# agussomacal/ROMHighContrast

Hardware: AMD Instinct MI355X
Metric: snapshot_solves_per_sec (higher is better)
Workload: dtype f64

## Files before the change

romhighcontrast_amd/csrc/rom_fem_kernels.hip:

```cpp
#include "rom_fem_dev.h"

__global__ void k_build_A0(double* A0, const double* Qp, const double* rho, int n1, int n1p, int N) {
  size_t idx = blockIdx.x * size_t(blockDim.x) + threadIdx.x;
  size_t total = size_t(n1) * n1 * n1p;
  if (idx >= total) return;
  int m = int(idx % n1p);
  size_t ij = idx / n1p;
  int j = int(ij % n1) + 1, i = int(ij / n1) + 1;
  A0[idx] = (m < n1) ? Qp[size_t(j - 1) * n1p + m] * rho[size_t(m) * (N + 1) + i] : 0.0;
}

__global__ void k_repack_table(const double* __restrict__ G, int ld, int nseg, int n1, int orient, double* __restrict__ Gs) {
  const long long idx = blockIdx.x * (long long)blockDim.x + threadIdx.x;
  const long long hrows = (long long)n1 * n1;
  if (idx >= (long long)nseg * hrows * 8) return;
  const int kk = int(idx & 7);
  const long long rp = (idx >> 3) % hrows, seg = (idx >> 3) / hrows;
  const long long row = orient ? (rp % n1) * n1 + rp / n1 : rp;
  const int k = int(seg) * 8 + kk;
  Gs[idx] = k < ld ? G[row * ld + k] : 0.0;
}

__global__ void k_mask_table(double* __restrict__ G, int ld, int n1, ExtThresholds th) {
  const long long idx = blockIdx.x * (long long)blockDim.x + threadIdx.x;
// ... 854 lines not shown
  const int m_raw = 4 * int(blockIdx.x) + w;
  const bool live = m_raw < Mc;
  const int m = live ? m_raw : Mc - 1;
  const double* am = a + size_t(m) * f.kblk;
  double* ym = f.y + size_t(m) * f.nGp;
#ifdef ROMHC_SOLVE1_STAMPS
  unsigned long long stamp[10];
#define S1_STAMP(i) stamp[i] = __builtin_readcyclecounter()
  S1_STAMP(0);
#else
#define S1_STAMP(i)
#endif
#define S1_WAVE_SYNC()                                   \
  do {                                                   \
    asm volatile("s_waitcnt lgkmcnt(0)" ::: "memory");   \
    __builtin_amdgcn_wave_barrier();                     \
  } while (0)
#define S1_BARRIER() asm volatile("s_waitcnt lgkmcnt(0)\n\ts_barrier" ::: "memory")
  const int l16 = lane & 15, l4 = lane >> 4;

  if (upd) {
    int4 irec[6], crec[S1_ITEM_PASSES];
    int wd[DENSE_GROUPS_MAX];
    {
      const int4* ir = reinterpret_cast<const int4*>(f.s1_items) + size_t(min(lane, max(f.ndi, 1) - 1)) * 6;
#pragma unroll
      for (int x = 0; x < 6; ++x) irec[x] = ir[x];
#pragma unroll
      for (int r = 0; r < S1_ITEM_PASSES; ++r) crec[r] = reinterpret_cast<const int4*>(f.s1_citems)[min(lane + 64 * r, max(f.ncoef, 1) - 1)];
#pragma unroll
      for (int g = 0; g < DENSE_GROUPS_MAX; ++g) wd[g] = g < f.ndg ? f.dweight[g * 64 + lane] : -2;
    }
    const int xr_first = lane < f.ncross ? f.xred[lane] : 0;
    const int2 sc_b = lane < f.nsc ? reinterpret_cast<const int2*>(f.scb)[lane] : int2{0, 0};
    const RhsTerm rt = f.rhs[min(lane, max(f.nrhs, 1) - 1)];
    const double gvec = f.g[lane];
    __syncthreads();
    {
      const double rcoef = lane < f.nrhs ? (rt.kind == 0 ? aL[rt.b0] / (aL[rt.e0] + aL[rt.e1]) : 0.5) : 0.0;
      double y = gvec;
      for (int t0 = 0; t0 < f.nrhs; t0 += 8) {
        double rv[8];
#pragma unroll
        for (int x = 0; x < 8; ++x) {
          rv[x] = 0.0;
          if (t0 + x < f.nrhs) {
            const int pos = __builtin_amdgcn_readlane(rt.pos, t0 + x), len = __builtin_amdgcn_readlane(rt.len, t0 + x);
            const int voff = __builtin_amdgcn_readlane(rt.voff, t0 + x);
            if (lane >= pos && lane < pos + len) rv[x] = f.vec[voff + lane - pos];
          }
        }
#pragma unroll
        for (int x = 0; x < 8; ++x)
          if (t0 + x < f.nrhs) y += readlane_f64(rcoef, t0 + x) * rv[x];
      }
      zs[lane] = y;
    }
    if (live)
      for (int i = lane; i < f.nGp; i += 64) ym[i] = 0.0;
    if (live && lane < f.nsc) ym[f.spos0 + lane] = sc_b.y >= 0 ? 1.0 / (aL[sc_b.x] + aL[sc_b.y]) : (1.0 / (double(f.N) * double(f.N))) / aL[sc_b.x];
    for (int i = lane + 64; live && i < f.nsc; i += 64) {
      const int b0 = f.scb[2 * i], b1 = f.scb[2 * i + 1];
      ym[f.spos0 + i] = b1 >= 0 ? 1.0 / (aL[b0] + aL[b1]) : (1.0 / (double(f.N) * double(f.N))) / aL[b0];
    }
    double wgt[DENSE_GROUPS_MAX];
#pragma unroll
    for (int g = 0; g < DENSE_GROUPS_MAX; ++g) {
      wgt[g] = 0.0;
      if (g < f.ndg) {
        const DenseGroup& dg = f.dgroups[g];
        wgt[g] = wd[g] >= 0 ? aL[wd[g]] : (wd[g] == -1 ? (aL[dg.b0] + aL[dg.b1]) / 2 : 0.0);
      }
    }
    const bool has_it = lane < f.ndi;
    const int it_g = irec[0].x, it_pos = irec[0].y, it_nv = irec[0].z;
    double it_den = 1.0, it_cv[4] = {0.0, 0.0, 0.0, 0.0}, it_vv[4] = {0.0, 0.0, 0.0, 0.0};
    if (has_it) {
      const int voff[4] = {irec[1].y, irec[1].z, irec[1].w, irec[2].x}, vblk[4] = {irec[2].y, irec[2].z, irec[2].w, irec[3].x};
      const int vu0[4] = {irec[3].y, irec[3].z, irec[3].w, irec[4].x}, vu1[4] = {irec[4].y, irec[4].z, irec[4].w, irec[5].x};
      it_den = aL[irec[0].w] + aL[irec[1].x];
#pragma unroll
      for (int v = 0; v < 4; ++v)
        if (v < it_nv) {
          it_cv[v] = aL[vblk[v]] / (aL[vu0[v]] + aL[vu1[v]]);
          it_vv[v] = f.vec[voff[v]];
        }
    }
    int ci_dst[S1_ITEM_PASSES], ci_src[S1_ITEM_PASSES];
#pragma unroll
    for (int r = 0; r < S1_ITEM_PASSES; ++r) {
      ci_src[r] = -1;
      ci_dst[r] = crec[r].x & 0xfffffff;
      if (lane + 64 * r < f.ncoef) {
        const int code = crec[r].x >> 28;
        if (code == 2) ci_src[r] = crec[r].y;
        else if (code != 0 && live) ym[ci_dst[r]] = code == 1 ? 1.0 / (aL[crec[r].z] + aL[crec[r].w]) : 0.0;
      }
    }
    __syncthreads();
    d4_t C[4][4];
    {
      int q = 0;
#pragma unroll
      for (int ib = 0; ib < 4; ++ib)
#pragma unroll
        for (int jb = 0; jb <= ib; ++jb, ++q)
#pragma unroll
          for (int g = 0; g < 4; ++g) {
            const int R = 16 * ib + 4 * g + l4, Cc = 16 * jb + l16;
            const double x = Ls[(q * 4 + g) * 64 + lane];
            C[ib][jb][g] = (R >= f.s1_ndr || Cc >= f.s1_ndr) ? (R == Cc ? 1.0 : 0.0) : x;
          }
    }
#pragma unroll
    for (int x = 0; x < 8; ++x) PnB[x * 64 + lane] = 0.0;
    S1_BARRIER();
#ifdef ROMHC_SOLVE1_PANEL_STAMPS
    unsigned long long uwait = 0;
    const unsigned long long ut0 = __builtin_readcyclecounter();
#endif
#pragma unroll
    for (int p = 0; p < 15; ++p) {
      const int jb = p >> 2;
      {
        const int p1 = p + 1, jb1 = p1 >> 2, co1 = 4 * (p1 & 3);
        double* dstp = PnB + (p1 & 1) * 256;
        if ((l16 >> 2) == (p1 & 3)) {
#pragma unroll
          for (int ib = jb1; ib < 4; ++ib)
#pragma unroll
            for (int g = 0; g < 4; ++g) dstp[(16 * ib + 4 * g + l4) * 4 + (l16 - co1)] = C[ib][jb1][g];
        }
      }
#ifdef ROMHC_SOLVE1_PANEL_STAMPS
      { const unsigned long long t0_ = __builtin_readcyclecounter(); S1_BARRIER(); uwait += __builtin_readcyclecounter() - t0_; }
#else
      S1_BARRIER();
#endif
      const double* Pp = (p & 1) ? Pn1 : Pn;
      double frag[4];
#pragma unroll
      for (int x = jb; x < 4; ++x) frag[x] = Pp[(16 * x + l16) * 4 + l4];
#pragma unroll
      for (int jb2 = jb; jb2 < 4; ++jb2)
#pragma unroll
        for (int ib = jb2; ib < 4; ++ib)
          C[ib][jb2] = __builtin_amdgcn_mfma_f64_16x16x4f64(-frag[ib], frag[jb2], C[ib][jb2], 0, 0, 0);
    }
#ifdef ROMHC_SOLVE1_PANEL_STAMPS
    const unsigned long long ut1 = __builtin_readcyclecounter();
#endif
    S1_BARRIER();
    if (!live) return;
    const double z = zs[lane];
    ym[lane] = z;
    if (lane < f.ncross) ym[f.xb0 + lane] = zs[xr_first];
    for (int x = lane + 64; x < f.ncross; x += 64) ym[f.xb0 + x] = zs[f.xred[x]];
#pragma unroll
    for (int g = 0; g < DENSE_GROUPS_MAX; ++g)
      if (g < f.ndg) wz[g * 64 + lane] = wgt[g] * z;
    S1_WAVE_SYNC();
    if (has_it) {
      const double* wg = wz + it_g * 64;
      const double* D = Dl + lane;
      double acc = 0.0;
#pragma unroll 1
      for (int j0 = 0; j0 < 64; j0 += 16) {
#pragma unroll
        for (int j = 0; j < 16; ++j) acc += D[(j0 + j) * f.ndi] * wg[j0 + j];
      }
#pragma unroll
      for (int v = 0; v < 4; ++v)
        if (v < it_nv) acc += it_cv[v] * it_vv[v];
      ym[it_pos] = acc / it_den;
    }
#pragma unroll
    for (int r = 0; r < S1_ITEM_PASSES; ++r)
      if (ci_src[r] >= 0) ym[ci_dst[r]] = zs[ci_src[r]];
    for (int it = lane + 64 * S1_ITEM_PASSES; it < f.ncoef; it += 64) {
      const CoefGroup& cg = f.groups[f.item_group[it]];
      const int k = f.item_k[it];
      if (cg.kind == 1 && k < cg.r) continue;
      ym[cg.cpos + k] = k == cg.r ? 1.0 / (aL[cg.b0] + aL[cg.b1]) : (k < cg.r ? zs[cg.zpos + k] : 0.0);
    }
#ifdef ROMHC_SOLVE1_STAMPS
    if (lane < 12) ym[lane] = PnB[lane];
#ifdef ROMHC_SOLVE1_PANEL_STAMPS
    if (lane == 12) ym[12] = double(uwait);
    if (lane == 13) ym[13] = double(ut1 - ut0);
#endif
#endif
    return;
  }

  {
    const unsigned d0 = unsigned(size_t((__attribute__((address_space(3))) char*)s1_dyn)) + unsigned(S1_COEF_BYTES + 4 * S1_WAVE_BYTES);
    const int nchunk = (f.ndi + 1) >> 1;
    const char* src = reinterpret_cast<const char*>(f.dmat);
    for (int c = w; c < nchunk; c += 4)
      asm volatile("s_mov_b32 m0, %0\n\tglobal_load_lds_dwordx4 %1, %2" ::"s"(__builtin_amdgcn_readfirstlane(d0 + unsigned(c) * 1024u)),
                   "v"(unsigned(lane) * 16u), "s"(x128_uniform(src + size_t(c) * 1024))
                   : "memory", "m0");
  }
  {
    const int p0 = f.wp0[w], np = f.wp0[w + 1] - p0;
    const double2* pbase = reinterpret_cast<const double2*>(f.pool_acc) + size_t(p0) * 128 + lane;
    double2 v[PAIR_RING][2];
    auto issue = [&](int i, double2 (&dst)[2]) {
      dst[0] = pbase[size_t(i) * 128];
      dst[1] = pbase[size_t(i) * 128 + 64];
    };
    const double a_l = lane < f.kblk ? am[lane] : 1.0;
    const GenTerm gt = f.terms[f.s1_t0 + min(lane, f.s1_nterm - 1)];
    int mine = f.wmeta[p0 + lane];
#pragma unroll
    for (int u = 0; u < PAIR_RING; ++u) issue(u, v[u]);
#pragma unroll
    for (int x = 0; x < 40; ++x) Ls[x * 64 + lane] = 0.0;
    aL[lane] = a_l;
    S1_WAVE_SYNC();
    coefs[w * 64 + lane] = lane < f.s1_nterm ? term_coef(gt, aL) : 0.0;
    __syncthreads();
    double cf[4];
#pragma unroll
    for (int s = 0; s < 4; ++s) cf[s] = coefs[s * 64 + lane];
    double acc4[4][4];
#pragma unroll
    for (int s = 0; s < 4; ++s)
#pragma unroll
      for (int g = 0; g < 4; ++g) acc4[s][g] = 0.0;
    double* const Cl0 = reinterpret_cast<double*>(s1_dyn + S1_COEF_BYTES) + lane;
    S1_STAMP(1);
    for (int base = 0; base < np; base += 64) {
      const int cur = mine;
      const int nxt = f.wmeta[p0 + base + 64 + lane];
      const int cnt = min(64, np - base);
#pragma unroll
      for (int i0 = 0; i0 < 64; i0 += PAIR_RING) {
        if (i0 >= cnt) break;
#pragma unroll
        for (int u = 0; u < PAIR_RING; ++u) {
          const int i = i0 + u;
          const int meta = __builtin_amdgcn_readlane(cur, i);
#pragma unroll
          for (int s = 0; s < 4; ++s) {
            const double c = readlane_f64(cf[s], meta & 0xff);
            acc4[s][0] = __builtin_fma(c, v[u][0].x, acc4[s][0]);
            acc4[s][1] = __builtin_fma(c, v[u][0].y, acc4[s][1]);
            acc4[s][2] = __builtin_fma(c, v[u][1].x, acc4[s][2]);
            acc4[s][3] = __builtin_fma(c, v[u][1].y, acc4[s][3]);
          }
          if (meta >> 16) {
            double* dst = Cl0 + ((meta >> 8) & 0xff) * 256;
#pragma unroll
            for (int s = 0; s < 4; ++s)
#pragma unroll
              for (int g = 0; g < 4; ++g) {
                dst[s * (S1_WAVE_BYTES / 8) + g * 64] = acc4[s][g];
                acc4[s][g] = 0.0;
              }
          }
          issue(base + i + PAIR_RING, v[u]);
        }
      }
      mine = nxt;
    }
    asm volatile("s_waitcnt vmcnt(0)" ::: "memory");
    __syncthreads();
  }
  S1_STAMP(2);
  double nv[4];
  {
    const int ib = lane >> 4;
    const double* src = Ls + ((ib * (ib + 1) / 2) * 4 + ((lane >> 2) & 3)) * 64 + (lane & 3) * 16;
    const double2 x0 = *reinterpret_cast<const double2*>(src), x1 = *reinterpret_cast<const double2*>(src + 2);
    nv[0] = x0.x; nv[1] = x0.y; nv[2] = x1.x; nv[3] = x1.y;
#pragma unroll
    for (int k = 0; k < 4; ++k)
      if (lane >= f.s1_ndr || k >= f.s1_ndr) nv[k] = lane == k ? 1.0 : 0.0;
  }
  S1_BARRIER();
  S1_STAMP(3);
  double y = zs[lane];
  double myrs = 0.0;
#ifdef ROMHC_SOLVE1_PANEL_STAMPS
  unsigned long long fwait = 0;
#endif
  S1_STAMP(4);
#pragma unroll
  for (int p = 0; p < 16; ++p) {
    const int c0 = 4 * p;
    chol_panel_regs(lane, c0, nv, y, myrs);
    {
      double* Pp = (p & 1) ? Pn1 : Pn;
      *reinterpret_cast<double2*>(&Pp[lane * 4]) = double2{nv[0], nv[1]};
      *reinterpret_cast<double2*>(&Pp[lane * 4 + 2]) = double2{nv[2], nv[3]};
    }
    if ((lane >> 2) >= p) {
      double* lrow = Ls + s1_lrow(lane) + c0;
      *reinterpret_cast<double2*>(lrow) = double2{nv[0], nv[1]};
      *reinterpret_cast<double2*>(lrow + 2) = double2{nv[2], nv[3]};
    }
    if (p < 15) {
#ifdef ROMHC_SOLVE1_PANEL_STAMPS
      { const unsigned long long t0_ = __builtin_readcyclecounter(); S1_BARRIER(); fwait += __builtin_readcyclecounter() - t0_; }
#else
      S1_BARRIER();
#endif
      const double* bp = PnB + ((p + 1) & 1) * 256 + lane * 4;
      const double2 b01 = *reinterpret_cast<const double2*>(bp), b23 = *reinterpret_cast<const double2*>(bp + 2);
      double nn[4] = {b01.x, b01.y, b23.x, b23.y};
#pragma unroll
      for (int kk = 0; kk < 4; ++kk)
#pragma unroll
        for (int k = 0; k < 4; ++k) nn[kk] = __builtin_fma(-nv[k], readlane_f64(nv[k], c0 + 4 + kk), nn[kk]);
#pragma unroll
      for (int kk = 0; kk < 4; ++kk) nv[kk] = nn[kk];
    }
  }
  if (chol_pivots_bad(myrs) && live && lane == 0) atomicOr(f.status, 1);
  S1_WAVE_SYNC();
  S1_STAMP(5);
#pragma unroll
  for (int h = 1; h >= 0; --h) {
    double lcol[32];
#pragma unroll
    for (int j = 0; j < 32; ++j) lcol[j] = Ls[s1_lrow(32 * h + j) + lane];
#pragma unroll
    for (int j = 31; j >= 0; --j) {
      const int jj = 32 * h + j;
      const double xj = readlane_f64(y, jj) * readlane_f64(myrs, jj);
      if (lane == jj) y = xj;
      else if (lane < jj) y -= lcol[j] * xj;
    }
  }
  zs[lane] = y;
  S1_STAMP(6);
#ifdef ROMHC_SOLVE1_STAMPS
#pragma unroll
  for (int k = 0; k < 7; ++k)
    if (lane == k) PnB[k] = double(stamp[k] - stamp[0]);
  if (lane >= 7 && lane < 12) PnB[lane] = 0.0;
#ifdef ROMHC_SOLVE1_PANEL_STAMPS
  if (lane == 10) PnB[10] = double(fwait);
#endif
#endif
  S1_BARRIER();
#undef S1_STAMP
#undef S1_WAVE_SYNC
#undef S1_BARRIER
}

template <int NS>
__device__ inline void panel_body(const FemDev& f, const double* __restrict__ am0, int m0, int nsys, int j, int ent, double* lds,
                                  double* yj, double* coef) {
  double* Cb = lds;
  double* stB = lds + TILE_DOUBLES;
  const int slot = f.colrow[ent];
  const int ti = f.colti[ent];
  const WavePos wp;
  const TileDesc& d = f.desc[slot];
  const int t = threadIdx.x;
  const bool stream = NS == 1 && f.tile_stream && d.t1 - d.t0 <= 128;
  STile st[NS];
  if (!stream) s_tile_load<NS>(st, d, f, am0, nsys, coef);
  static_assert(TD_LDS_BYTES <= FACT_LDS_DOUBLES * 8, "the DMA slots alias the staging area and the C tile");
#pragma unroll
  for (int q = 0; q < NS; ++q) {
    if (q >= nsys) break;
    const int m = m0 + q;
    double* Lm = f.L + size_t(m) * f.nslots * 4096;
    if (q > 0) __syncthreads();
    if (t < 64) yj[t] = f.y[size_t(m) * f.nGp + j * 64 + t];
    TileStream<1> ts;
    if (stream) s_tile_stream_begin<1>(ts, slot, d, f, am0 + size_t(q) * f.kblk, 1);
    Acc acc;
    acc_zero(acc);
    accumulate_klist_dma(f, slot, Lm, [](int) { return true; }, acc, reinterpret_cast<char*>(lds), wp);
    if (stream) {
      __syncthreads();
      double* T[1] = {Cb};
      s_tile_to_lds<1>(T, ts, d, f);
      tile_minus_acc(Cb, acc, wp);
    } else {
      tile_from_acc(Cb, acc, st[q], wp);
    }

    acc_zero(acc);
    const double* I = f.invL + (size_t(m) * f.T + j) * 4096 + (t >> 2) * 64 + (t & 3) * 2;
    const int kmax = (wp.wc + 1) * 32;
    {
      const int fr = wp.lane & 15, kq = wp.lane >> 4;
      double2 vb = *reinterpret_cast<const double2*>(I);
      for (int ch = 0; ch < 8; ++ch) {
        *reinterpret_cast<double2*>(stB + (t >> 2) * LDK8 + (t & 3) * 2) = vb;
        __syncthreads();
        if (ch + 1 < 8) vb = *reinterpret_cast<const double2*>(I + (ch + 1) * 8);
        if (ch * 8 < kmax) {
          const double* pa = Cb + (wp.wr * 32 + fr) * LDC + ch * 8 + kq;
          const double* pb = stB + (wp.wc * 32 + fr) * LDK8 + kq;
#pragma unroll
          for (int kk = 0; kk < 8; kk += 4) {
            const double a0 = pa[kk], a1 = pa[16 * LDC + kk];
            const double b0 = pb[kk], b1 = pb[16 * LDK8 + kk];
            acc.c[0][0] = __builtin_amdgcn_mfma_f64_16x16x4f64(a0, b0, acc.c[0][0], 0, 0, 0);
            acc.c[0][1] = __builtin_amdgcn_mfma_f64_16x16x4f64(a0, b1, acc.c[0][1], 0, 0, 0);
            acc.c[1][0] = __builtin_amdgcn_mfma_f64_16x16x4f64(a1, b0, acc.c[1][0], 0, 0, 0);
            acc.c[1][1] = __builtin_amdgcn_mfma_f64_16x16x4f64(a1, b1, acc.c[1][1], 0, 0, 0);
          }
        }
        __syncthreads();
      }
    }

    double* Lout = Lm + size_t(slot) * 4096;
#pragma unroll
    for (int i = 0; i < 2; ++i)
#pragma unroll
      for (int jb = 0; jb < 2; ++jb)
#pragma unroll
        for (int g = 0; g < 4; ++g) {
          int r = acc_row(wp, i, g), c = acc_col(wp, jb);
          double v = acc.c[i][jb][g];
          Lout[r * 64 + c] = v;
          Cb[r * LDC + c] = v;
        }
    __syncthreads();
    if (t < 64) {
      double sum = 0.0;
      for (int k = 0; k < 64; ++k) sum += Cb[t * LDC + k] * yj[k];
      f.y[size_t(m) * f.nGp + ti * 64 + t] -= sum;
    }
  }
}

__device__ inline void panel_block(int b, int nrows, int Mc, int& m, int& row) {
  const int xcd = b & 7, idx = b >> 3;
  const int full = (Mc >> 3) << 3;
  m = xcd + 8 * (idx / nrows);
  row = idx % nrows;
  if (m >= full) {
    const int tb = b - full * nrows;
    m = full + tb / nrows;
    row = tb % nrows;
  }
}

template <int NS>
__global__ __launch_bounds__(256, 4) void k_factor_panel(FemDev f, const double* __restrict__ a, int j, int Mc) {
  __shared__ __align__(16) double lds[FACT_LDS_DOUBLES];
  __shared__ double yj[64];
  double* coef = lds;
  int mp, row;
  panel_block(blockIdx.x, f.colptr[j + 1] - f.colptr[j], (Mc + NS - 1) / NS, mp, row);
  const int m0 = mp * NS;
  panel_body<NS>(f, a + size_t(m0) * f.kblk, m0, min(NS, Mc - m0), j, f.colptr[j] + row, lds, yj, coef);
}
template __global__ void k_factor_panel<1>(FemDev, const double*, int, int);

__global__ __launch_bounds__(256) void k_backsolve(FemDev f) {
  extern __shared__ __align__(16) double xs[];
  __shared__ double red[4][64];
  __shared__ double vs[64];
  const int m = blockIdx.x;
  const int t = threadIdx.x, c = t & 63, part = t >> 6;
  const double* Lm = f.L + size_t(m) * f.nslots * 4096;
  double* ym = f.y + size_t(m) * f.nGp;
  for (int j = f.T - 1; j >= 0; --j) {
    double s = 0.0;
    for (int e = f.colptr[j]; e < f.colptr[j + 1]; ++e) {
      const double* Lt = Lm + size_t(f.colrow[e]) * 4096;
      const double* xi = xs + f.colti[e] * 64;
#pragma unroll 4
      for (int rr = part * 16; rr < part * 16 + 16; ++rr) s += Lt[rr * 64 + c] * xi[rr];
    }
    red[part][c] = s;
    __syncthreads();
    if (t < 64) vs[t] = ym[j * 64 + t] - (red[0][t] + red[1][t] + red[2][t] + red[3][t]);
    __syncthreads();
    const double* It = f.invL + (size_t(m) * f.T + j) * 4096;
    s = 0.0;
#pragma unroll 4
    for (int rr = part * 16; rr < part * 16 + 16; ++rr) s += It[rr * 64 + c] * vs[rr];
    red[part][c] = s;
    __syncthreads();
    if (t < 64) xs[j * 64 + t] = red[0][t] + red[1][t] + red[2][t] + red[3][t];
    __syncthreads();
  }
  for (int v = t; v < f.nGa; v += 256) ym[v] = xs[v];
}

__global__ __launch_bounds__(256) void k_edge_transform(FemDev f, int Mc) {
  __shared__ __align__(16) double lds[STAGE_TOTAL];
  const WavePos wp;
  const int pos = f.epos[blockIdx.z];
  const int srow = stage_row(), sseg = stage_seg();
  const int mA = blockIdx.y * 64 + srow;
  const double* pA = mA < Mc ? f.y + size_t(mA) * f.nGp + pos + sseg : nullptr;
  const double* pB = f.Qp + size_t(blockIdx.x * 64 + srow) * f.n1p + sseg;
  Acc acc;
  acc_zero(acc);
  gemm_loop(
      f.n1p / BK, [&](int ch, double* v) { load4_aligned(pA ? pA + ch * BK : nullptr, v); },
      [&](int ch, double* v) { load4_aligned(pB + ch * BK, v); }, acc, lds, wp);
#pragma unroll
  for (int i = 0; i < 2; ++i)
#pragma unroll
    for (int g = 0; g < 4; ++g) {
      const int m = blockIdx.y * 64 + acc_row(wp, i, g);
      if (m >= Mc) continue;
#pragma unroll
      for (int jb = 0; jb < 2; ++jb)
        f.yhat[size_t(m) * f.nGp + pos + blockIdx.x * 64 + acc_col(wp, jb)] = acc.c[i][jb][g];
    }
}


__global__ __launch_bounds__(256) void k_extend(FemDev f, const double* __restrict__ a, int Mc,
                                                double* __restrict__ U, long long row0, const int* __restrict__ blocks,
                                                int pw_log2) {
  __shared__ __align__(16) double lds[STAGE_TOTAL];
  __shared__ double scs[64];
  double* stage = lds;
  const WavePos wp;
  const int b = blocks[blockIdx.z];
  const int p = b / f.ncb, q = b % f.ncb;
  const int n1 = f.n1, N = f.N;
  const BlockSide& sd = f.sides[b];
  const int srow = stage_row(), sseg = stage_seg();
  const int pw = 1 << pw_log2, ph = 64 >> pw_log2;
  const int npj = (n1 + pw - 1) >> pw_log2;
  const int pi = blockIdx.x / npj, pj = blockIdx.x % npj;
  const int i0 = ph * pi + 1, j0 = pw * pj + 1;
  const int i1 = min(i0 + ph - 1, n1), j1 = min(j0 + pw - 1, n1);

  const int mA = blockIdx.y * 64 + srow;
  const bool vA = mA < Mc;
  const int iB = i0 + (srow >> pw_log2), jB = j0 + (srow & (pw - 1));
  const bool vB = iB <= n1 && jB <= n1;

  int cend[4];
  const double* pAs[4];
  const double* pBs[4];
  int tot = 0;
#pragma unroll
  for (int s = 0; s < 4; ++s) {
    const ExtSide es = sd.s[s];
    int nch = 0;
    pAs[s] = pBs[s] = nullptr;
    if (es.mode != 0) {
      const int hrow = vB ? h0_row(s, iB, jB, N, n1) : 0;
      if (es.mode == 1) {
        const int dist = s == 0 ? i0 : s == 1 ? N - i1 : s == 2 ? j0 : N - j1;
        nch = f.kmax[dist] / BK;
        if (vA) pAs[s] = f.yhat + size_t(mA) * f.nGp + es.off + sseg;
        if (vB) pBs[s] = f.A0 + size_t(hrow) * f.n1p + sseg;
      } else {
        nch = es.nch;
        if (vA) pAs[s] = f.y + size_t(mA) * f.nGp + es.off + sseg;
        if (vB) pBs[s] = f.G + es.gtab + size_t(hrow) * (es.nch * BK) + sseg;
      }
    }
    tot += nch;
    cend[s] = tot;
  }
  if (threadIdx.x < 64) {
    const int m = blockIdx.y * 64 + threadIdx.x;
    scs[threadIdx.x] = m < Mc ? f.y[size_t(m) * f.nGp + f.sblk0 + b] : 0.0;
  }
  __syncthreads();
  Acc acc;
  acc_zero(acc);
  auto pick = [&](int ch, const double* const* ps) -> const double* {
    const int s = (ch >= cend[0]) + (ch >= cend[1]) + (ch >= cend[2]);
    const int lc = ch - (s == 0 ? 0 : s == 1 ? cend[0] : s == 2 ? cend[1] : cend[2]);
    const double* p = s == 0 ? ps[0] : s == 1 ? ps[1] : s == 2 ? ps[2] : ps[3];
    return p ? p + lc * BK : nullptr;
  };
  gemm_loop(
      tot, [&](int ch, double* v) { load4_aligned(pick(ch, pAs), v); },
      [&](int ch, double* v) { load4_aligned(pick(ch, pBs), v); }, acc, stage, wp);

  const bool odd = wp.lane & 1;
  const int cfirst = acc_col(wp, odd ? 1 : 0) - (odd ? 1 : 0);
  const int ii = i0 + (cfirst >> pw_log2) - 1, jj = j0 + (cfirst & (pw - 1)) - 1;
  const bool v0 = ii < n1 && jj < n1, v1 = ii < n1 && jj + 1 < n1;
  const long long gidx = (long long)(p * N + ii) * f.nc + (q * N + jj);
  double w_own[2];
#pragma unroll
  for (int jb = 0; jb < 2; ++jb) {
    const int cidx = acc_col(wp, jb);
    const int wi = i0 + (cidx >> pw_log2) - 1, wj = j0 + (cidx & (pw - 1)) - 1;
    w_own[jb] = (wi < n1 && wj < n1) ? f.W[wi * n1 + wj] : 0.0;
  }
#pragma unroll
  for (int i = 0; i < 2; ++i)
#pragma unroll
    for (int g = 0; g < 4; ++g) {
      const int m = blockIdx.y * 64 + acc_row(wp, i, g);
      const double sc = scs[acc_row(wp, i, g)];
      const double x0 = acc.c[i][0][g] + sc * w_own[0], x1 = acc.c[i][1][g] + sc * w_own[1];
      const double got = lane_swap1(odd ? x0 : x1);
      if (m >= Mc) continue;
      double* dst = U + (row0 + m) * f.dim + gidx;
      const double lo = odd ? got : x0, hi = odd ? x1 : got;
      if (v1) *reinterpret_cast<double2_u*>(dst) = double2_u{lo, hi};
      else if (v0) dst[0] = lo;
    }
}



constexpr int X128_SLOT = 4 * 128 * 64;
static_assert(sizeof(FemDev) + sizeof(X128Args) + 64 <= 4096, "k_extend128's arguments must fit the kernel argument segment");

template <bool FLAT>
__global__ __launch_bounds__(512, 2) void k_extend128(FemDev f, X128Args xa, const double* __restrict__ a, int Mc,
                                                      double* __restrict__ U, long long row0, int with_expand,
                                                      int sys_fast, int wave_skip) {
  __shared__ __align__(16) char lds_bytes[2 * X128_SLOT];
  __shared__ double scs[128];
  double* const lds = reinterpret_cast<double*>(lds_bytes);
  const int n1 = f.n1, N = f.N;
  const int nct = (n1 + 127) / 128;
  const int nvert = n1 * n1;
  const int ntile = FLAT ? (nvert + 127) / 128 : n1 * nct;
  int bx, by, ngy;
  if (sys_fast > 0) {
    bx = int(blockIdx.x) / sys_fast; by = int(blockIdx.x) % sys_fast; ngy = sys_fast;
  } else if (sys_fast < 0) {
    ngy = -sys_fast;
    const int unit = int(blockIdx.x) / (8 * ngy), r = int(blockIdx.x) % (8 * ngy);
    bx = unit * 8 + (r & 7); by = r >> 3;
  } else {
    bx = int(blockIdx.x); by = int(blockIdx.y); ngy = int(gridDim.y);
  }
// ... 306 lines not shown
```

Baseline: 4.456 million.

## Read Cholesky panel from LDS and block the back-substitution by four

The Schur update in the panel Cholesky now takes the next panel's values from the shared-memory panel buffer, loaded before the barrier, instead of through cross-lane readlane broadcasts. The backward triangular solve is restructured into 4-column blocks. Each block solves its 4x4 diagonal triangle from L entries and reciprocal pivots that are staged in shared memory and prefetched one block ahead. This cuts the serial readlane chain roughly fourfold, at the cost of extra LDS reads and more register pressure.

Result: no change. 4.486 million, median of 5 (+0.7%).

```diff
diff --git a/romhighcontrast_amd/csrc/rom_fem_kernels.hip b/romhighcontrast_amd/csrc/rom_fem_kernels.hip
--- a/romhighcontrast_amd/csrc/rom_fem_kernels.hip
+++ b/romhighcontrast_amd/csrc/rom_fem_kernels.hip
@@ -1180,6 +1180,15 @@
       *reinterpret_cast<double2*>(lrow + 2) = double2{nv[2], nv[3]};
     }
     if (p < 15) {
+      double2 un[4][2];
+      {
+        const double* Pp = (p & 1) ? Pn1 : Pn;
+#pragma unroll
+        for (int kk = 0; kk < 4; ++kk) {
+          un[kk][0] = *reinterpret_cast<const double2*>(&Pp[(c0 + 4 + kk) * 4]);
+          un[kk][1] = *reinterpret_cast<const double2*>(&Pp[(c0 + 4 + kk) * 4 + 2]);
+        }
+      }
 #ifdef ROMHC_SOLVE1_PANEL_STAMPS
       { const unsigned long long t0_ = __builtin_readcyclecounter(); S1_BARRIER(); fwait += __builtin_readcyclecounter() - t0_; }
 #else
@@ -1189,27 +1198,53 @@
       const double2 b01 = *reinterpret_cast<const double2*>(bp), b23 = *reinterpret_cast<const double2*>(bp + 2);
       double nn[4] = {b01.x, b01.y, b23.x, b23.y};
 #pragma unroll
-      for (int kk = 0; kk < 4; ++kk)
-#pragma unroll
-        for (int k = 0; k < 4; ++k) nn[kk] = __builtin_fma(-nv[k], readlane_f64(nv[k], c0 + 4 + kk), nn[kk]);
+      for (int kk = 0; kk < 4; ++kk) {
+        const double uk[4] = {un[kk][0].x, un[kk][0].y, un[kk][1].x, un[kk][1].y};
+#pragma unroll
+        for (int k = 0; k < 4; ++k) nn[kk] = __builtin_fma(-nv[k], uk[k], nn[kk]);
+      }
 #pragma unroll
       for (int kk = 0; kk < 4; ++kk) nv[kk] = nn[kk];
     }
   }
   if (chol_pivots_bad(myrs) && live && lane == 0) atomicOr(f.status, 1);
+  zs[lane] = myrs;
   S1_WAVE_SYNC();
   S1_STAMP(5);
+  struct BsPanel { double l10, l32; double2 l2, l3, r01, r23; };
+  auto bs_fetch = [&](int c0) {
+    BsPanel b;
+    b.l10 = Ls[s1_lrow(c0 + 1) + c0];
+    b.l2 = *reinterpret_cast<const double2*>(&Ls[s1_lrow(c0 + 2) + c0]);
+    b.l3 = *reinterpret_cast<const double2*>(&Ls[s1_lrow(c0 + 3) + c0]);
+    b.l32 = Ls[s1_lrow(c0 + 3) + c0 + 2];
+    b.r01 = *reinterpret_cast<const double2*>(&zs[c0]);
+    b.r23 = *reinterpret_cast<const double2*>(&zs[c0 + 2]);
+    return b;
+  };
+  BsPanel bn = bs_fetch(60);
 #pragma unroll
   for (int h = 1; h >= 0; --h) {
     double lcol[32];
 #pragma unroll
     for (int j = 0; j < 32; ++j) lcol[j] = Ls[s1_lrow(32 * h + j) + lane];
 #pragma unroll
-    for (int j = 31; j >= 0; --j) {
-      const int jj = 32 * h + j;
-      const double xj = readlane_f64(y, jj) * readlane_f64(myrs, jj);
-      if (lane == jj) y = xj;
-      else if (lane < jj) y -= lcol[j] * xj;
+    for (int q = 7; q >= 0; --q) {
+      const int c0 = 32 * h + 4 * q;
+      const BsPanel b = bn;
+      if (c0 > 0) bn = bs_fetch(c0 - 4);
+      double y0 = readlane_f64(y, c0), y1 = readlane_f64(y, c0 + 1), y2 = readlane_f64(y, c0 + 2);
+      const double x3 = readlane_f64(y, c0 + 3) * b.r23.y;
+      y2 -= b.l32 * x3; y1 -= b.l3.y * x3; y0 -= b.l3.x * x3;
+      const double x2 = y2 * b.r23.x;
+      y1 -= b.l2.y * x2; y0 -= b.l2.x * x2;
+      const double x1 = y1 * b.r01.y;
+      y0 -= b.l10 * x1;
+      const double x0 = y0 * b.r01.x;
+      double t = y;
+      t -= lcol[4 * q + 3] * x3; t -= lcol[4 * q + 2] * x2; t -= lcol[4 * q + 1] * x1; t -= lcol[4 * q] * x0;
+      const double xk = (lane & 3) == 0 ? x0 : ((lane & 3) == 1 ? x1 : ((lane & 3) == 2 ? x2 : x3));
+      y = lane < c0 ? t : ((lane >> 2) == (c0 >> 2) ? xk : y);
     }
   }
   zs[lane] = y;
```
